# casys-kaist/CoVA

Measured on AMD Instinct MI355X. Metric: compressed-domain frames/sec (BlobNet+bboxcc) at 1080p b=256, higher is better.
Workload: dtype f16

## Files before the change

cova_amd/csrc/blobnet.h:

```cpp
#pragma once
#include <hip/hip_fp16.h>

#include <vector>

#include "internal.h"

constexpr int BN_T = 4;
constexpr int BN_LEVELS = 4;
constexpr int BN_KTAB_STACKS = 256;

struct BnLevelGeom {
    int H, W;
};

struct BnWorkspace {
    bool ready = false;
    __half *act[BN_LEVELS + 1] = {};
    __half *dact[BN_LEVELS] = {};
    __half *pbuf = nullptr;
    size_t pbuf_frames = 0;
    float *part = nullptr;
    int32_t *d_index = nullptr;
    int32_t *h_index = nullptr;
    size_t index_ints = 0;
// ... 6 lines not shown
    hipEvent_t ev_models = nullptr;
    std::vector<uint8_t> last_models;
    int32_t *d_areas = nullptr;
    int32_t *h_areas = nullptr;
    size_t areas_cap = 0;
    hipEvent_t ev_areas = nullptr;
    std::vector<int32_t> last_areas;
};

struct covahip_blobnet {
    int H = 0, W = 0, max_batch = 0;
    int n_models = 1;
    BnLevelGeom lv[BN_LEVELS + 1];
    int enc_c[BN_LEVELS + 1] = {3, 16, 32, 64, 128};
    int dec_ci[BN_LEVELS] = {128, 128, 64, 32};
    int dec_co[BN_LEVELS] = {64, 32, 16, 16};
    int dec_cy[BN_LEVELS], dec_cx[BN_LEVELS];
    BnWorkspace ws[COVAHIP_MAX_LANES];
    void *d_prepared = nullptr;
    size_t prepared_bytes = 0;
    struct Prepared *prep = nullptr;
    int fuse_tail = 1;
    int fuse_dec = 1;
    int enc1_tile16 = 1;
    int tail_rows = 1;
    int tail_part = 1;
    int fuse_enc23 = 1;
    int enc_rowtiles = 1;
    int64_t macs_per_frame = 0;
    std::vector<float> post_thr;
    std::vector<int32_t> post_area;
    bool area_on = false;
    std::vector<std::vector<uint8_t>> post_keep;
    bool post_on = false;
    void *d_post = nullptr;
    size_t post_area_off = 0, post_keep_off = 0, post_planes_off = 0, post_keep_stride = 0, post_planes_stride = 0, post_bytes = 0;
};

constexpr int BN_E1_MAXW = 62;
inline bool bn_level1_on_enc1(const covahip_ctx *ctx, const covahip_blobnet *m) {
    return m->enc1_tile16 && m->enc_c[1] == 16 && m->enc_c[2] == 32 && m->lv[1].W <= BN_E1_MAXW && m->lv[1].H >= 2 &&
           !ctx->enc_plan[1].nbands;
}

int blobnet_prepare_mfma(covahip_ctx *ctx, covahip_blobnet *m, const float *const *h_weights, int n_models);
void blobnet_release_mfma(covahip_ctx *ctx, covahip_blobnet *m);
// ... 22 lines not shown
```

cova_amd/csrc/blobnet.hip:

```cpp
#include <algorithm>
#include <cmath>
#include <cstdlib>
#include <cstring>
#include <vector>

#include "blobnet.h"
#include "covahip_dev.h"

namespace {

constexpr uint32_t W_MAGIC = 0x57485643;
constexpr size_t N_PARAMS = 320305;

}

static void free_model(covahip_ctx *ctx, covahip_blobnet *m) {
    if (!m) return;
    blobnet_release_mfma(ctx, m);
    if (m->d_post) hipFree(m->d_post);
    for (BnWorkspace &ws : m->ws) {
        for (int i = 0; i <= BN_LEVELS; i++)
            if (ws.act[i]) hipFree(ws.act[i]);
        for (int j = 0; j < BN_LEVELS; j++)
            if (ws.dact[j]) hipFree(ws.dact[j]);
// ... 452 lines not shown
        const size_t hw = (size_t)m->H * m->W;
        if (keep.empty()) std::memset(keep_or_null, 1, hw);
        else std::memcpy(keep_or_null, keep.data(), hw);
    }
    return COVAHIP_OK;
}

int covahip_blobnet_macs_per_frame(covahip_ctx *ctx, int64_t *macs) {
    if (!ctx || !macs) return COVAHIP_ERR_INVALID_ARG;
    if (!ctx->blobnet) return COVAHIP_ERR_NOT_LOADED;
    *macs = ctx->blobnet->macs_per_frame;
    return COVAHIP_OK;
}

int covahip_blobnet_set_enc_plan(covahip_ctx *ctx, int level, int nbands, int nbuf) {
    if (!ctx || level < 1 || level > 3 || nbands < 0 || nbands > 64 || (nbands && nbuf != 1 && nbuf != 2)) return COVAHIP_ERR_INVALID_ARG;
    ctx->enc_plan[level].nbands = nbands;
    ctx->enc_plan[level].nbuf = nbands ? nbuf : 0;
    return COVAHIP_OK;
}

int covahip_blobnet_set_impl(covahip_ctx *ctx, int impl) {
    if (!ctx || !ctx->blobnet) return COVAHIP_ERR_NOT_LOADED;
    if (impl != 1 && (impl < 4 || impl > 10)) return COVAHIP_ERR_INVALID_ARG;
    ctx->blobnet->fuse_dec = impl != 4;
    ctx->blobnet->enc1_tile16 = impl != 5;
    ctx->blobnet->enc_rowtiles = impl != 6;
    ctx->blobnet->fuse_enc23 = impl == 7 ? 0 : impl == 8 ? 2 : 1;
    ctx->blobnet->tail_part = impl != 9;
    ctx->blobnet->tail_rows = impl != 10;
    return COVAHIP_OK;
}

static int filter_placed(covahip_ctx *ctx, covahip_blobnet *m, const uint8_t *d_src, int n_frames, const int32_t *stack_index,
                         int batch, int area_thresh, covahip_box *d_boxes, int32_t *d_counts, int max_boxes, float *d_logits,
                         uint8_t *d_mask, bool packed = false, const uint8_t *model_ids = nullptr) {
    if (!d_mask) {
        CtxLane &l = ctx->lane();
        int rc = covahip_ensure_buffer(ctx, &l.cc_scratch, &l.cc_scratch_bytes, (size_t)batch * m->H * m->W);
        if (rc) return rc;
        d_mask = (uint8_t *)l.cc_scratch;
    }
    BnInput in;
    if (n_frames > 0) {
        int rc = prepare_frames(ctx, m, m->ws[ctx->cur_lane], d_src, n_frames, stack_index, batch, in, model_ids);
        if (rc) return rc;
        in.packed = packed;
    } else {
        in.stack = d_src;
    }
    return filter_dev(ctx, in, batch, d_logits, d_mask, true, area_thresh, d_boxes, d_counts, max_boxes, n_frames > 0 ? nullptr : model_ids);
}

// ... 235 lines not shown
```

cova_amd/csrc/blobnet_mfma.hip:

```cpp
#include <algorithm>
#include <cmath>
#include <cstdlib>
#include <cstring>
#include <mutex>
#include <type_traits>
#include <utility>
#include <vector>

#include "bboxcc_body.h"
#include "bboxcc_wave.h"
#include "blobnet.h"
#include "covahip_dev.h"

typedef _Float16 half8 __attribute__((ext_vector_type(8)));
typedef _Float16 half4 __attribute__((ext_vector_type(4)));
typedef float f32x16 __attribute__((ext_vector_type(16)));
typedef float f32x4 __attribute__((ext_vector_type(4)));
typedef _Float16 half2v __attribute__((ext_vector_type(2)));

namespace {

constexpr float BN_EPS = 1e-3f;
constexpr int WG = 256;

// ... 1112 lines not shown
            const uint4 sv = *reinterpret_cast<const uint4 *>(scr + ll * 16);
            if (owin < nwin) {
                const int owy = fdiv(owin, p.mWp), owx = owin - owy * p.Wp;
                const int gy = y0 / 2 + owy + p.oy, gx = owx + p.ox;
                const uint32_t eo = (uint32_t)((gy * p.Wo + gx) * 32 + 8 * (m & 3));
                *reinterpret_cast<uint4 *>(ob + (m >> 2) * tstride + eo) = sv;
                if (ride && m < 4) {
                    float *const pw = reinterpret_cast<float *>(pb4 + (y0 + 2 * owy) * GW + 2 * owx) + m;
                    pw[0] = pride[0]; pw[4] = pride[1]; pw[4 * GW] = pride[2]; pw[4 * GW + 4] = pride[3];
                }
            }
            __builtin_amdgcn_fence(__ATOMIC_RELEASE, "wavefront");
            __builtin_amdgcn_wave_barrier();
            PHASE_MARK(7);
        }
    }
#ifdef PHASE_TIMING
    if (tid == 64 * (PHASE_WAVE < 0 ? NWV + PHASE_WAVE : PHASE_WAVE))
        for (int i = 0; i < 9; i++) atomicAdd(&g_phase[i], ph_[i]);
#endif
    WGSPAN_END(0);
}

constexpr int E23_RP2 = 2048;
constexpr int E23_NSLOT = 6;
constexpr int E23_TSZ2 = E23_NSLOT * E23_RP2;
struct Enc23Args {
    const __half *in;
    __half *mid;
    __half *out;
    const half8 *wf2, *wf3;
    const float *epi2, *epi3;
    int B;
    int H2, W2, Hp2, Wp2;
    int H3, W3, Hp3, Wp3, oy3, ox3;
    int H4, W4, oy4, ox4;
    Swz swz2, swz3;
    int ring_off, xchg_off, scr_off;
    const uint8_t *model_ids;
    uint32_t mstride;
};
template <bool AP2, bool AP3, bool MS = false>
__global__ __launch_bounds__(512, 2) void enc23_mfma(Enc23Args p) {
    extern __shared__ __attribute__((aligned(256))) uint8_t smem[];
    WGSPAN_BEGIN();
    const int tid = threadIdx.x, lane = tid & 63;
    const int wave = __builtin_amdgcn_readfirstlane(tid >> 6);
    uint8_t *const ring = smem + p.ring_off;
    uint8_t *const xchg = smem + p.xchg_off;
    const int TC3 = p.W3 + 2;
    bool first = true;
    const int tc2 = wave & 1, nt2 = (wave >> 1) & 1, th = wave >> 2;
    const int nt3 = wave & 3, mg3 = wave >> 2;
    for (int b = blockIdx.x; b < p.B; b += gridDim.x) {
        [[maybe_unused]] const uint32_t moff = model_off<MS>(p.model_ids, p.mstride, b);
        int ll = lane;
        asm volatile("" : "+v"(ll));
        lds_barrier();
        const uint8_t *const src_b = reinterpret_cast<const uint8_t *>(p.in) + (size_t)b * BN_T * p.H2 * p.W2 * 64;
        const int st_t = tid >> 7, st_i = tid & 127, st_c = st_i >> 2, st_x = st_c - 1;
        const bool st_xin = st_x >= 0 && st_x < p.W2;
        uint32_t st_so[2];
#pragma unroll
        for (int k = 0; k < 2; k++)
            st_so[k] = (uint32_t)((min(max(st_x, 0), p.W2 - 1)) * 64 + (((st_i & 3) ^ swz_eval<4>(p.swz2, st_c, k)) << 4));
// ... 5 lines not shown
                const int rc = min(max(r0 + k, 0), p.H2 - 1);
                v[k] = *reinterpret_cast<const uint4 *>(st_src + (size_t)rc * p.W2 * 64 + st_so[k]);
            }
        };
        auto store_rows = [&](int r0, const uint4 (&v)[2]) {
#pragma unroll
            for (int k = 0; k < 2; k++) {
                const int row = r0 + k;
                const bool in = st_xin && row >= 0 && row < p.H2;
                *reinterpret_cast<uint4 *>(st_dst + ((row + 1) % E23_NSLOT) * E23_RP2) = in ? v[k] : make_uint4(0, 0, 0, 0);
            }
        };
        {
            uint4 va[2], vb[2];
            load_rows(-1, va);
            load_rows(1, vb);
            if (first) {
                for (int i = tid; i < BN_T * E3_TSZ / 16; i += 512) *reinterpret_cast<uint4 *>(smem + i * 16) = make_uint4(0, 0, 0, 0);
                first = false;
            }
            store_rows(-1, va);
            store_rows(1, vb);
        }
        {
            const int m0 = ll & 31, kh = ll >> 5;
            const int yl = (m0 >> 1) & 1, xl = 2 * (m0 >> 2) + (m0 & 1);
            uint32_t xq2[9];
#pragma unroll
            for (int tap = 0; tap < 9; tap++) {
                const int yy = yl + tap / 3, xx = xl + 16 * tc2 + tap % 3;
                xq2[tap] = (uint32_t)(p.ring_off + th * 2 * E23_TSZ2 + xx * 64) ^ (uint32_t)((kh ^ swz_eval<4>(p.swz2, xx, yy)) << 4);
            }
            half8 bf[18];
            {
                const half8 *wp = at_model(p.wf2, moff) + nt2 * 18 * 64 + ll;
                asm volatile("" : "+v"(wp));
#pragma unroll
                for (int ks = 0; ks < 18; ks++) bf[ks] = wp[ks * 64];
            }
            const int co = nt2 * 32 + (ll & 31);
            const float *const epi2 = at_model(p.epi2, moff);
            const float e0 = epi2[co], e1 = epi2[64 + co], e2 = epi2[128 + co];
            const TmixW tm = load_tmix(epi2 + 192, ll);
            int s0 = 0;
            for (int s = 0; s < p.Hp2; s++) {
                lds_barrier();
                uint4 vn[2];
                const bool pre = s + 1 < p.Hp2;
                if (pre) load_rows(2 * s + 3, vn);
                uint32_t fa[9];
                {
#pragma unroll
                    for (int ty = 0; ty < 3; ty++) {
                        int slot = s0 + ty + yl;
                        slot = slot >= E23_NSLOT ? slot - E23_NSLOT : slot;
                        const uint32_t rr = (uint32_t)(slot * E23_RP2);
#pragma unroll
                        for (int tx = 0; tx < 3; tx++) fa[ty * 3 + tx] = xq2[ty * 3 + tx] + rr;
                    }
                }
                s0 = s0 + 2 >= E23_NSLOT ? s0 + 2 - E23_NSLOT : s0 + 2;
                constexpr int AD = 8, NS = 36;
                auto frag = [&](int i) -> half8 {
                    const int tap = i >> 2, kc = (i >> 1) & 1, t = i & 1;
                    const uint8_t *a = smem + (fa[tap] ^ (uint32_t)(kc << 5));
                    return *reinterpret_cast<const half8 *>(__builtin_assume_aligned(a + t * E23_TSZ2, 16));
                };
                half8 ab[AD];
#pragma unroll
                for (int i = 0; i < AD; i++) ab[i] = frag(i);
                f32x16 acc[2];
#pragma unroll
                for (int i = 0; i < NS; i++) {
                    const int t = i & 1;
                    if (i < 2) {
#pragma unroll
                        for (int q = 0; q < 16; q++) acc[t][q] = 0.f;
                    }
                    acc[t] = __builtin_amdgcn_mfma_f32_32x32x16_f16(ab[i % AD], bf[i >> 1], acc[t], 0, 0, 0);
                    if (i + AD < NS) ab[i % AD] = frag(i + AD);
                }
                __builtin_amdgcn_sched_group_barrier(0x100, AD, 0);
#pragma unroll
                for (int i = 0; i < NS; i++) {
                    __builtin_amdgcn_sched_group_barrier(0x008, 1, 0);
                    if (i + AD < NS) __builtin_amdgcn_sched_group_barrier(0x100, 1, 0);
                }
                half2v hp[4];
#pragma unroll
                for (int g = 0; g < 4; g++)
#pragma unroll
                    for (int t = 0; t < 2; t++)
                        hp[g][t] = (_Float16)pool4<AP2>(acc[t][4 * g], acc[t][4 * g + 1], acc[t][4 * g + 2], acc[t][4 * g + 3], e0, e1, e2);
                {
                    typedef _Float16 half4x __attribute__((ext_vector_type(4)));
                    const half4x give = th ? half4x{hp[0][0], hp[0][1], hp[1][0], hp[1][1]} : half4x{hp[2][0], hp[2][1], hp[3][0], hp[3][1]};
                    *reinterpret_cast<half4x *>(xchg + (wave * 64 + ll) * 8) = give;
                }
                if (pre) store_rows(2 * s + 3, vn);
                lds_barrier();
                half4 pb[2], o[2];
                {
                    const half4 got = *reinterpret_cast<const half4 *>(xchg + ((wave ^ 4) * 64 + ll) * 8);
                    if (th == 0) {
                        pb[0] = half4{hp[0][0], hp[0][1], got[0], got[1]};
                        pb[1] = half4{hp[1][0], hp[1][1], got[2], got[3]};
                    } else {
                        pb[0] = half4{got[0], got[1], hp[2][0], hp[2][1]};
                        pb[1] = half4{got[2], got[3], hp[3][0], hp[3][1]};
                    }
                }
                tmix4h<2>(tm, pb, o);
#pragma unroll
                for (int gl = 0; gl < 2; gl++) {
                    const int owx = 8 * tc2 + 2 * (2 * th + gl) + kh;
                    if (owx < p.Wp2) {
                        const int yy = s + p.oy3 + 1, xx = owx + p.ox3 + 1;
                        uint8_t *d = smem + (yy * TC3 + xx) * 128 + ((((co >> 3) ^ swz_eval<8>(p.swz3, xx, yy))) << 4) + (co & 7) * 2;
#pragma unroll
                        for (int t = 0; t < BN_T; t++) *reinterpret_cast<_Float16 *>(d + t * E3_TSZ) = o[gl][t];
                    }
                }
            }
        }
        {
            int l3 = lane;
            asm volatile("" : "+v"(l3));
            const int m0 = l3 & 31, kh = l3 >> 5;
            const int yl = (m0 >> 1) & 1, xl = 2 * (m0 >> 2) + (m0 & 1);
            half8 bf[36];
            {
                const half8 *wp = at_model(p.wf3, moff) + nt3 * 36 * 64 + ll;
                asm volatile("" : "+v"(wp));
#pragma unroll
                for (int ks = 0; ks < 36; ks++) bf[ks] = wp[ks * 64];
            }
            lds_barrier();
            {
                __half *const mb = p.mid + (size_t)b * BN_T * p.H3 * p.W3 * 64;
                const int npc = p.Hp2 * p.Wp2 * 8;
                for (int i = tid; i < npc; i += 512) {
                    const int pix = i >> 3, j = i & 7;
                    const int wy = pix / p.Wp2, wx = pix - wy * p.Wp2;
                    const int yy = wy + p.oy3 + 1, xx = wx + p.ox3 + 1;
                    const uint4 v = *reinterpret_cast<const uint4 *>(smem + (yy * TC3 + xx) * 128 + ((j ^ swz_eval<8>(p.swz3, xx, yy)) << 4));
                    *reinterpret_cast<uint4 *>(mb + ((size_t)(yy - 1) * p.W3 + (xx - 1)) * 64 + j * 8) = v;
                }
            }
            const int co = nt3 * 32 + (ll & 31);
            const float *const epi3 = at_model(p.epi3, moff);
            const float e0 = epi3[co], e1 = epi3[128 + co], e2 = epi3[256 + co];
            const TmixW tm = load_tmix(epi3 + 384, ll);
            uint32_t kq[9];
#pragma unroll
            for (int tap = 0; tap < 9; tap++) {
                const int yy = yl + tap / 3, xx = xl + tap % 3;
                kq[tap] = (uint32_t)((yy * TC3 + xx) * 128) ^ (uint32_t)((kh ^ swz_eval<8>(p.swz3, xx, yy)) << 4);
            }
// ... 274 lines not shown
template <int C1, int C2>
__device__ __forceinline__ void dec012_stage(uint8_t *tile, const __half *ss, const DecLvl &g, int wave, int lane, int first) {
    constexpr int C = C1 + C2, CPP = C / 8;
    const int RC = (g.Wi + 2) * CPP, NI = g.Wi * CPP;
    for (int y = (wave + 8 - first) & 7; y < g.Hi; y += 8) {
        const int r = y + 1;
        const __half *rowp = ss + (size_t)y * g.Wi * C2;
        uint8_t *rowl = tile + (r * RC + CPP) * 16;
        for (int q0 = 0; q0 < NI; q0 += 64) {
            const int q = q0 + lane;
            const int px = q / CPP, chp = q % CPP;
            const int cb = (chp ^ swz_eval<CPP>(g.swz, px + 1, r)) * 8;
            if (q < NI && cb >= C1) glds16(rowp + px * C2 + (cb - C1), rowl + q0 * 16);
        }
    }
}

template <int C, int COUT>
struct Dec012W {
    half8 wf[4 * (C / 16)];
    float es[16], eb[16];
};
template <int C, int COUT>
__device__ __forceinline__ void dec012_load(Dec012W<C, COUT> &w, const half8 *wfrag, const float *epi, int wave, int lane) {
    constexpr int MT = 4 * COUT / 32, KSTEPS = 4 * (C / 16);
    const int mtile = wave % MT, kh = lane >> 5;
    asm volatile("" : "+s"(wfrag), "+s"(epi));
#pragma unroll
    for (int ks = 0; ks < KSTEPS; ks++) w.wf[ks] = wfrag[(mtile * KSTEPS + ks) * 64 + lane];
#pragma unroll
    for (int gq = 0; gq < 4; gq++) {
        const int c0 = (mtile * 32 + 8 * gq + 4 * kh) % COUT;
        const float4 sc = *reinterpret_cast<const float4 *>(epi + c0), sh = *reinterpret_cast<const float4 *>(epi + COUT + c0);
        w.es[4 * gq] = sc.x; w.es[4 * gq + 1] = sc.y; w.es[4 * gq + 2] = sc.z; w.es[4 * gq + 3] = sc.w;
        w.eb[4 * gq] = sh.x; w.eb[4 * gq + 1] = sh.y; w.eb[4 * gq + 2] = sh.z; w.eb[4 * gq + 3] = sh.w;
    }
}
template <int C1, int C2, int COUT, int CN>
__device__ __forceinline__ void dec012_block(const uint8_t *lds0, const uint8_t *tile, uint8_t *next_tile, __half *gout, uint8_t *scr_base,
                                             const Dec012W<C1 + C2, COUT> &w, const DecLvl &g, const DecLvl &gn,
                                             int wave, int lane) {
    constexpr int C = C1 + C2, MT = 4 * COUT / 32, PG = 8 / MT;
    constexpr int KC = C / 16, KSTEPS = 4 * KC, CPP = C / 8, PS = C * 2;
    constexpr int AD = C == 128 ? 4 : 8;
    const int mtile = wave % MT, pgroup = wave / MT;
    const int TC = g.Wi + 2, GW = g.Wi + 1, GH = g.Hi + 1;
    const int kh = lane >> 5;
    const half8 (&wf)[KSTEPS] = w.wf;
    const float (&es)[16] = w.es, (&eb)[16] = w.eb;
    const int npos = GH * GW;
    const int ntiles = (npos + 31) / 32;
    for (int tile_i = pgroup; tile_i < ntiles; tile_i += PG) {
        const int q = tile_i * 32 + (lane & 31);
        const int qc = min(q, npos - 1);
        const int u = fdiv(qc, g.mGW), v = qc - u * GW;
        const uint32_t toff = (uint32_t)(uintptr_t)(lds_void *)tile;
        uint32_t pk[4];
#pragma unroll
// ... 3 lines not shown
        }
        auto frag = [&](int ks) -> half8 {
            const int tp = ks / KC, kc = ks % KC;
            typedef const __attribute__((address_space(3))) half8 *lds_half8_ptr;
            return *(lds_half8_ptr)(uintptr_t)(pk[tp] ^ (uint32_t)(kc << 5));
        };
        half8 ring[AD];
#pragma unroll
        for (int ks = 0; ks < AD; ks++) ring[ks] = frag(ks);
        f32x16 acc;
#pragma unroll
        for (int r = 0; r < 16; r++) acc[r] = 0.f;
#pragma unroll
        for (int ks = 0; ks < KSTEPS; ks++) {
            acc = __builtin_amdgcn_mfma_f32_32x32x16_f16(wf[ks], ring[ks % AD], acc, 0, 0, 0);
            if (ks + AD < KSTEPS) ring[ks % AD] = frag(ks + AD);
        }
        __builtin_amdgcn_sched_group_barrier(0x100, AD, 0);
#pragma unroll
        for (int ks = 0; ks < KSTEPS; ks++) {
            __builtin_amdgcn_sched_group_barrier(0x008, 1, 0);
            if (ks + AD < KSTEPS) __builtin_amdgcn_sched_group_barrier(0x100, 1, 0);
        }
        if constexpr (CN > 0) {
            constexpr int CPPN = CN / 8, PSN = CN * 2;
            const int TCN = gn.Wi + 2;
            static_assert(COUT >= 32 && COUT % 32 == 0, "one output pixel per lane and tile");
            const int nb = mtile * 32 + 4 * kh;
            const int phase = nb / COUT, cob = nb % COUT;
            const int Y = 2 * u + (phase >> 1) - g.cy, X = 2 * v + (phase & 1) - g.cx;
            if (q < npos && Y >= 0 && Y < g.Hd && X >= 0 && X < g.Wd) {
                const int yy = Y + 1, xx = X + 1;
                uint8_t *const pix = next_tile + (yy * TCN + xx) * PSN + (cob & 7) * 2;
                const int sw = swz_eval<CPPN>(gn.swz, xx, yy);
#pragma unroll
                for (int gq = 0; gq < 4; gq++) {
                    half4 o;
#pragma unroll
                    for (int j = 0; j < 4; j++)
                        o[j] = (_Float16)fmaxf(acc[4 * gq + j] * es[4 * gq + j] + eb[4 * gq + j], 0.f);
                    *reinterpret_cast<half4 *>(pix + ((((cob >> 3) + gq) ^ sw) * 16)) = o;
                }
            }
        } else {
            uint8_t *const scr = scr_base + wave * 2048;
            const int pos = lane & 31;
#pragma unroll
            for (int gq = 0; gq < 4; gq++) {
                half4 o;
#pragma unroll
                for (int j = 0; j < 4; j++) o[j] = (_Float16)fmaxf(acc[4 * gq + j] * es[4 * gq + j] + eb[4 * gq + j], 0.f);
                *reinterpret_cast<half4 *>(scr + pos * 64 + ((gq ^ ((pos >> 2) & 3)) * 16) + kh * 8) = o;
            }
            __builtin_amdgcn_fence(__ATOMIC_RELEASE, "wavefront");
            __builtin_amdgcn_wave_barrier();
            __builtin_amdgcn_fence(__ATOMIC_ACQUIRE, "wavefront");
#pragma unroll
            for (int j = 0; j < 2; j++) {
                const int c = j * 64 + lane;
                const int rp = c >> 2;
                const int gq = (c & 3) ^ ((rp >> 2) & 3);
                const int rq = tile_i * 32 + rp;
                if (rq < npos) {
                    const int ru = fdiv(rq, g.mGW), rv = rq - ru * GW;
                    const int n0 = mtile * 32 + 8 * gq;
                    const int phase = n0 / COUT, co0 = n0 % COUT;
                    const int Y = 2 * ru + (phase >> 1) - g.cy, X = 2 * rv + (phase & 1) - g.cx;
                    if (Y >= 0 && Y < g.Hd && X >= 0 && X < g.Wd)
                        *reinterpret_cast<uint4 *>(gout + ((size_t)Y * g.Wd + X) * COUT + co0) =
                            *reinterpret_cast<const uint4 *>(scr + c * 16);
                }
            }
            __builtin_amdgcn_fence(__ATOMIC_RELEASE, "wavefront");
            __builtin_amdgcn_wave_barrier();
        }
    }
}

template <bool MS = false>
__global__ __launch_bounds__(512, 2) void dec012_mfma(Dec012Args p) {
    extern __shared__ __attribute__((aligned(256))) uint8_t smem[];
    const int tid = threadIdx.x, lane = tid & 63, wave = tid >> 6;
    uint8_t *const t0 = smem + p.lv[0].tile_off, *const t1 = smem + p.lv[1].tile_off, *const t2 = smem + p.lv[2].tile_off;
    WGSPAN_BEGIN();
#ifdef PHASE_TIMING
    unsigned long long ph_[9] = {0, 0, 0, 0, 0, 0, 0, 0, 0}, last_ = __builtin_amdgcn_s_memrealtime();
#endif
    dec012_zero_border<128>(t0, p.lv[0], tid);
    dec012_zero_border<128>(t1, p.lv[1], tid);
    dec012_zero_border<64>(t2, p.lv[2], tid);
    for (int b = blockIdx.x; b < p.B; b += gridDim.x) {
        [[maybe_unused]] const uint32_t moff = model_off<MS>(p.model_ids, p.mstride, b);
        if (b != (int)blockIdx.x) lds_barrier();
        PHASE_MARK(0);
        {
            Dec012W<128, 64> w0;
            dec012_load(w0, at_model(p.wf[0], moff), at_model(p.epi[0], moff), wave, lane);
            dec012_stage<0, 128>(t0, p.skip[0] + (size_t)b * p.Ts[0] * p.lv[0].Hi * p.lv[0].Wi * 128, p.lv[0], wave, lane, 0);
            dec012_stage<64, 64>(t1, p.skip[1] + (size_t)b * p.Ts[1] * p.lv[1].Hi * p.lv[1].Wi * 64, p.lv[1], wave, lane, p.lv[0].Hi & 7);
            dec012_stage<32, 32>(t2, p.skip[2] + (size_t)b * p.Ts[2] * p.lv[2].Hi * p.lv[2].Wi * 32, p.lv[2], wave, lane,
                                 (p.lv[0].Hi + p.lv[1].Hi) & 7);
            PHASE_MARK(1);
            wait_vmem();
            lds_barrier();
            PHASE_MARK(2);
            dec012_block<0, 128, 64, 128>(smem, t0, t1, nullptr, nullptr, w0, p.lv[0], p.lv[1], wave, lane);
        }
        PHASE_MARK(3);
        {
            Dec012W<128, 32> w1;
            dec012_load(w1, at_model(p.wf[1], moff), at_model(p.epi[1], moff), wave, lane);
            lds_barrier();
#ifdef PHASE_TIMING
            asm volatile("s_waitcnt vmcnt(0)" ::: "memory");
#endif
            PHASE_MARK(4);
            dec012_block<64, 64, 32, 64>(smem, t1, t2, nullptr, nullptr, w1, p.lv[1], p.lv[2], wave, lane);
        }
        PHASE_MARK(5);
        {
            Dec012W<64, 16> w2;
            dec012_load(w2, at_model(p.wf[2], moff), at_model(p.epi[2], moff), wave, lane);
            lds_barrier();
#ifdef PHASE_TIMING
            asm volatile("s_waitcnt vmcnt(0)" ::: "memory");
#endif
            PHASE_MARK(6);
            dec012_block<32, 32, 16, 0>(smem, t2, nullptr, p.out + (size_t)b * p.lv[2].Hd * p.lv[2].Wd * 16, smem + p.scr_off, w2,
                                        p.lv[2], p.lv[2], wave, lane);
        }
        PHASE_MARK(7);
    }
#ifdef PHASE_TIMING
    if (tid == 0)
        for (int i = 0; i < 9; i++) atomicAdd(&g_phase[48 + i], ph_[i]);
#endif
    WGSPAN_END(3);
}

struct Dec3ccArgs {
    DecArgs d;
    ccbody::CcGeom g;
    ccwave::WvGeom wg;
    int use_wv;
    covahip_box *boxes;
    int32_t *counts;
    int area_thresh, max_boxes;
    int tile_bytes;
    int mfull_off, cc_off;
    int part_off;
    DecMs ms;
};
// ... 798 lines not shown
    const Prepared *pr = f.pr;
    if (!(m->fuse_enc23 && m->enc_rowtiles && !f.ctx->enc_plan[2].nbands && !f.ctx->enc_plan[3].nbands && m->enc_c[2] == 32 &&
          m->enc_c[3] == 64 && m->enc_c[4] == 128))
        return false;
    const int H = m->lv[2].H, W = m->lv[2].W, Hp = H / 2, Wp = W / 2;
    const int H3 = m->lv[3].H, W3 = m->lv[3].W, Hp3 = H3 / 2, Wp3 = W3 / 2;
    const size_t lds = (size_t)BN_T * E3_TSZ + (size_t)BN_T * E23_TSZ2 + 4096;
    const bool pays = 4 * f.batch >= 3 * f.num_cu && 20 * Wp >= 17 * 8 * ((Wp + 7) / 8) && 20 * Wp3 >= 17 * 8 * ((Wp3 + 7) / 8);
    if (!((pays || m->fuse_enc23 == 2 || f.ms) && (W + 2) * 64 <= E23_RP2 && Wp <= 16 && Hp >= 1 && Hp3 >= 1 && Wp3 >= 1 &&
          (size_t)std::max(2 * Hp3 + 2, H3 + 1) * (W3 + 2) * 128 <= (size_t)E3_TSZ && lds <= 160 * 1024 - 256))
        return false;
    Enc23Args a;
    a.in = f.ws.act[2]; a.mid = f.ws.act[3]; a.out = f.ws.act[4];
    a.wf2 = (const half8 *)(f.prep + pr->enc[2].wfrag); a.wf3 = (const half8 *)(f.prep + pr->enc[3].wfrag);
    a.epi2 = (const float *)(f.prep + pr->enc[2].epi); a.epi3 = (const float *)(f.prep + pr->enc[3].epi);
    a.B = f.batch;
    a.H2 = H; a.W2 = W; a.Hp2 = Hp; a.Wp2 = Wp;
    a.H3 = H3; a.W3 = W3; a.Hp3 = Hp3; a.Wp3 = Wp3; a.oy3 = H & 1; a.ox3 = W & 1;
    a.H4 = m->lv[4].H; a.W4 = m->lv[4].W; a.oy4 = H3 & 1; a.ox4 = W3 & 1;
    a.swz2 = choose_swz_periodic(32, 30, Wp); a.swz3 = choose_swz_periodic(64, W3, Wp3);
    a.ring_off = BN_T * E3_TSZ; a.xchg_off = a.ring_off + BN_T * E23_TSZ2; a.scr_off = a.ring_off;
    a.model_ids = f.inp.model_ids; a.mstride = f.mstride;
    const int grid = std::min(f.batch, f.num_cu);
    rc = launched(f, with_bools([&](auto AP2, auto AP3, auto MS) {
        return launch(f, "enc23_mfma", enc23_mfma<AP2.value, AP3.value, MS.value>, grid, 512, lds, a);
    }, pr->allpos[2], pr->allpos[3], f.ms));
    return true;
}

int run_enc_level(const Fwd &f, int i) {
    const covahip_blobnet *m = f.m;
    const Prepared *pr = f.pr;
    const int H = m->lv[i].H, W = m->lv[i].W, Hp = H / 2, Wp = W / 2;
    const int cin = m->enc_c[i];
    const size_t px_bytes = (size_t)cin * 2;
    const int TC = W + 2;
    static const int enc_waves[BN_LEVELS] = {0, 8, 4, 8};
    int nbuf = 1, wgs_per_cu = (i == BN_LEVELS - 1) ? 1 : 2;
    int nbands = 0;
    const size_t scr_bytes = (size_t)enc_waves[i] * 2048;
    if (f.ctx->enc_plan[i].nbands) {
        nbands = std::min(f.ctx->enc_plan[i].nbands, Hp);
        nbuf = f.ctx->enc_plan[i].nbuf;
        const size_t need = (size_t)nbuf * BN_T * (2 * ((Hp + nbands - 1) / nbands) + 2) * TC * px_bytes + scr_bytes;
        if (need > 160 * 1024 - 256) return COVAHIP_ERR_UNSUPPORTED;
        wgs_per_cu = (i == BN_LEVELS - 1) ? 1 : (int)std::min<size_t>(2, (160 * 1024 - 256) / need);
    } else {
        const size_t lds_cap = (wgs_per_cu == 1 ? 150 * 1024 : 80 * 1024) - scr_bytes;
        nbands = plan_bands(Hp, f.batch, (long long)wgs_per_cu * f.num_cu,
// ... 49 lines not shown
          m->dec_co[1] == 32 && m->dec_co[2] == 16))
        return false;
    Dec012Args a;
    size_t off = 0;
    for (int j = 0; j < 3; j++) {
        const BnLevelGeom in = m->lv[BN_LEVELS - j], out = m->lv[BN_LEVELS - 1 - j];
        DecLvl &g = a.lv[j];
        g.Hi = in.H; g.Wi = in.W; g.Hd = out.H; g.Wd = out.W; g.cy = m->dec_cy[j]; g.cx = m->dec_cx[j];
        g.mGW = magic(in.W + 1);
        g.mRC = magic((in.W + 2) * (m->dec_ci[j] / 8));
        g.swz = choose_swz(false, m->dec_ci[j], in.W, 0, in.H + 1);
        g.tile_off = (int)off;
        off += (((size_t)(in.H + 2) * (in.W + 2) * m->dec_ci[j] * 2) + 255) & ~(size_t)255;
        a.skip[j] = f.ws.act[BN_LEVELS - j];
        a.Ts[j] = j == 0 ? 1 : BN_T;
        a.wf[j] = (const half8 *)(f.prep + pr->dec[j].wfrag);
        a.epi[j] = (const float *)(f.prep + pr->dec[j].epi);
    }
    a.scr_off = (int)off;
    const size_t lds = off + 8 * 2048;
    if (lds > 160 * 1024 - 256) return false;
    a.out = f.ws.dact[2]; a.B = f.batch; a.zero = f.prep + pr->zero;
    a.model_ids = f.inp.model_ids; a.mstride = f.mstride;
    rc = launched(f, with_bools([&](auto MS) {
        return launch(f, "dec012_mfma", dec012_mfma<MS.value>, std::min(f.batch, f.num_cu), 512, lds, a);
    }, f.ms));
    return true;
}

struct DecPlan {
    DecArgs a;
    DecMs am;
    BnLevelGeom in, out;
    bool half;
    int ci, GH, grid;
    size_t row_bytes, lds;
};
int plan_dec_block(const Fwd &f, int j, DecPlan &p) {
    const covahip_blobnet *m = f.m;
    const Prepared *pr = f.pr;
    const BnLevelGeom in = m->lv[BN_LEVELS - j], out = m->lv[BN_LEVELS - 1 - j];
    const bool last = j == BN_LEVELS - 1;
    const bool half = last && f.part_written;
    const int ci_j = half ? m->dec_ci[j] / 2 : m->dec_ci[j];
    DecArgs &a = p.a;
    a.up = j == 0 ? nullptr : f.ws.dact[j - 1];
    a.skip = f.ws.act[BN_LEVELS - j];
    a.out = last ? nullptr : f.ws.dact[j];
    a.logits = last ? f.d_logits : nullptr;
// ... 188 lines not shown
```

cova_amd/elements.py:

```python
from __future__ import annotations

import ctypes as C

import numpy as np

from . import _lib as L
from . import weights as W

FLOW_OK = "ok"
FLOW_DROPPED = "dropped"


def _ptr(a: np.ndarray) -> int:
    return a.ctypes.data


def _optr(a: np.ndarray | None) -> int | None:
    return None if a is None else a.ctypes.data


class Context:

    def __init__(self, device_id: int = 0):
        self._lib = L.lib()
# ... 170 lines not shown

    def reset_post(self, model: int = 0):
        L.check(self._lib.covahip_blobnet_set_post(self.ctx.handle, model, None), "covahip_blobnet_set_post", self.ctx.handle)

    def post(self, model: int = 0):
        thr, has = C.c_float(), C.c_int()
        keep = np.empty((self.h, self.w), dtype=np.uint8)
        L.check(self._lib.covahip_blobnet_get_post(self.ctx.handle, model, C.byref(thr), _ptr(keep), C.byref(has)),
                "covahip_blobnet_get_post", self.ctx.handle)
        return thr.value, (keep if has.value else None)

    def set_area(self, model: int = 0, area: int = 0):
        L.check(self._lib.covahip_blobnet_set_area(self.ctx.handle, model, int(area)), "covahip_blobnet_set_area", self.ctx.handle)

    def get_area(self, model: int = 0) -> int:
        v = C.c_int()
        L.check(self._lib.covahip_blobnet_get_area(self.ctx.handle, model, C.byref(v)), "covahip_blobnet_get_area", self.ctx.handle)
        return v.value

    def set_enc_plan(self, level: int, nbands: int, nbuf: int = 1):
        L.check(self._lib.covahip_blobnet_set_enc_plan(self.ctx.handle, level, nbands, nbuf), "covahip_blobnet_set_enc_plan")

    def set_impl(self, impl: str):
        L.check(self._lib.covahip_blobnet_set_impl(self.ctx.handle, {"mfma": 1, "dec_separate": 4, "enc1_legacy": 5, "enc_general_tiles": 6, "enc23_separate": 7, "enc23_force": 8, "tail_skip_tensor": 9, "tail_band_tiles": 10}[impl]), "set_impl")

    TAIL_ALONE, TAIL_ROWS, TAIL_BANDS = 1, 2, 4

    def tail_form(self) -> int:
        v = C.c_int()
        L.check(self._lib.covahip_dev_blobnet_tail_form(self.ctx.handle, C.byref(v)), "covahip_dev_blobnet_tail_form")
        return v.value

    def read_buffer(self, which: int, index: int = 0) -> np.ndarray:
        p, n, dims = C.c_void_p(), C.c_size_t(), (C.c_int32 * 5)()
        L.check(self._lib.covahip_dev_blobnet_buffer(self.ctx.handle, which, index, C.byref(p), C.byref(n), dims),
                "covahip_dev_blobnet_buffer", self.ctx.handle)
        out = np.empty(tuple(d for d in dims if d), dtype=np.float32 if which == 3 else np.float16)
        assert p.value and out.nbytes == n.value, (which, index, n.value, tuple(dims))
        self.ctx.d2h(out, p.value)
        return out

    @property
    def macs_per_frame(self) -> int:
        v = C.c_int64()
        L.check(self._lib.covahip_blobnet_macs_per_frame(self.ctx.handle, C.byref(v)), "macs_per_frame")
        return v.value

# ... 526 lines not shown
```

Baseline: 2.424 million.

## Prefetch next decoder level weights into recycled registers during last tiles

In the fused decoder kernel, the weight-fragment registers of the current level are reused. While the final tiles of one level run, the next level's weight fragments are loaded into them with inline global loads, so the weight-load latency between levels is hidden. Tile processing now also handles two tiles per wave on the last pass, and the epilogue is factored into a helper. A similar register-recycling prefetch for enc23 is added behind a non-default option (impl 12). The price is fragile hand-written waitcnt and asm register pinning, plus higher register pressure.

```diff
diff --git a/cova_amd/csrc/blobnet.h b/cova_amd/csrc/blobnet.h
--- a/cova_amd/csrc/blobnet.h
+++ b/cova_amd/csrc/blobnet.h
@@ -52,6 +52,8 @@
     struct Prepared *prep = nullptr;
     int fuse_tail = 1;
     int fuse_dec = 1;
+    int dec_kouter = 1;
+    int enc23_recycle = 0;
     int enc1_tile16 = 1;
     int tail_rows = 1;
     int tail_part = 1;
diff --git a/cova_amd/csrc/blobnet.hip b/cova_amd/csrc/blobnet.hip
--- a/cova_amd/csrc/blobnet.hip
+++ b/cova_amd/csrc/blobnet.hip
@@ -498,13 +498,15 @@
 
 int covahip_blobnet_set_impl(covahip_ctx *ctx, int impl) {
     if (!ctx || !ctx->blobnet) return COVAHIP_ERR_NOT_LOADED;
-    if (impl != 1 && (impl < 4 || impl > 10)) return COVAHIP_ERR_INVALID_ARG;
+    if (impl != 1 && (impl < 4 || impl > 12)) return COVAHIP_ERR_INVALID_ARG;
     ctx->blobnet->fuse_dec = impl != 4;
     ctx->blobnet->enc1_tile16 = impl != 5;
     ctx->blobnet->enc_rowtiles = impl != 6;
-    ctx->blobnet->fuse_enc23 = impl == 7 ? 0 : impl == 8 ? 2 : 1;
+    ctx->blobnet->fuse_enc23 = impl == 7 ? 0 : impl == 8 || impl == 12 ? 2 : 1;
     ctx->blobnet->tail_part = impl != 9;
     ctx->blobnet->tail_rows = impl != 10;
+    ctx->blobnet->dec_kouter = impl != 11;
+    ctx->blobnet->enc23_recycle = impl == 12;
     return COVAHIP_OK;
 }
 
diff --git a/cova_amd/csrc/blobnet_mfma.hip b/cova_amd/csrc/blobnet_mfma.hip
--- a/cova_amd/csrc/blobnet_mfma.hip
+++ b/cova_amd/csrc/blobnet_mfma.hip
@@ -1158,6 +1158,7 @@
     WGSPAN_END(0);
 }
 
+__device__ __forceinline__ void dec012_recycle(half8 &f, uint32_t voff, const half8 *base, int ks);
 constexpr int E23_RP2 = 2048;
 constexpr int E23_NSLOT = 6;
 constexpr int E23_TSZ2 = E23_NSLOT * E23_RP2;
@@ -1176,7 +1177,7 @@
     const uint8_t *model_ids;
     uint32_t mstride;
 };
-template <bool AP2, bool AP3, bool MS = false>
+template <bool AP2, bool AP3, bool MS = false, bool RC = false>
 __global__ __launch_bounds__(512, 2) void enc23_mfma(Enc23Args p) {
     extern __shared__ __attribute__((aligned(256))) uint8_t smem[];
     WGSPAN_BEGIN();
@@ -1228,7 +1229,9 @@
             store_rows(-1, va);
             store_rows(1, vb);
         }
+        half8 bf2[18];
         {
+            half8 (&bf)[18] = bf2;
             const int m0 = ll & 31, kh = ll >> 5;
             const int yl = (m0 >> 1) & 1, xl = 2 * (m0 >> 2) + (m0 & 1);
             uint32_t xq2[9];
@@ -1237,7 +1240,6 @@
                 const int yy = yl + tap / 3, xx = xl + 16 * tc2 + tap % 3;
                 xq2[tap] = (uint32_t)(p.ring_off + th * 2 * E23_TSZ2 + xx * 64) ^ (uint32_t)((kh ^ swz_eval<4>(p.swz2, xx, yy)) << 4);
             }
-            half8 bf[18];
             {
                 const half8 *wp = at_model(p.wf2, moff) + nt2 * 18 * 64 + ll;
                 asm volatile("" : "+v"(wp));
@@ -1249,10 +1251,14 @@
             const float e0 = epi2[co], e1 = epi2[64 + co], e2 = epi2[128 + co];
             const TmixW tm = load_tmix(epi2 + 192, ll);
             int s0 = 0;
-            for (int s = 0; s < p.Hp2; s++) {
+            const half8 *wf3b = at_model(p.wf3, moff);
+            uint32_t voff3 = (uint32_t)((nt3 * 36 * 64 + ll) * 16);
+            asm volatile("" : "+s"(wf3b));
+            auto step = [&](int s, auto LAST) __attribute__((always_inline)) {
+                constexpr bool last = decltype(LAST)::value;
                 lds_barrier();
                 uint4 vn[2];
-                const bool pre = s + 1 < p.Hp2;
+                const bool pre = !last && s + 1 < p.Hp2;
                 if (pre) load_rows(2 * s + 3, vn);
                 uint32_t fa[9];
                 {
@@ -1285,12 +1291,18 @@
                     }
                     acc[t] = __builtin_amdgcn_mfma_f32_32x32x16_f16(ab[i % AD], bf[i >> 1], acc[t], 0, 0, 0);
                     if (i + AD < NS) ab[i % AD] = frag(i + AD);
-                }
-                __builtin_amdgcn_sched_group_barrier(0x100, AD, 0);
-#pragma unroll
-                for (int i = 0; i < NS; i++) {
-                    __builtin_amdgcn_sched_group_barrier(0x008, 1, 0);
-                    if (i + AD < NS) __builtin_amdgcn_sched_group_barrier(0x100, 1, 0);
+                    if (last && (i & 1)) {
+                        dec012_recycle(bf[i >> 1], voff3, wf3b, i >> 1);
+                        if (((i >> 1) & 3) == 3) voff3 += 4096;
+                    }
+                }
+                if constexpr (!last) {
+                    __builtin_amdgcn_sched_group_barrier(0x100, AD, 0);
+#pragma unroll
+                    for (int i = 0; i < NS; i++) {
+                        __builtin_amdgcn_sched_group_barrier(0x008, 1, 0);
+                        if (i + AD < NS) __builtin_amdgcn_sched_group_barrier(0x100, 1, 0);
+                    }
                 }
                 half2v hp[4];
 #pragma unroll
@@ -1327,6 +1339,12 @@
                         for (int t = 0; t < BN_T; t++) *reinterpret_cast<_Float16 *>(d + t * E3_TSZ) = o[gl][t];
                     }
                 }
+            };
+            if constexpr (RC) {
+                for (int s = 0; s + 1 < p.Hp2; s++) step(s, std::false_type{});
+                step(p.Hp2 - 1, std::true_type{});
+            } else {
+                for (int s = 0; s < p.Hp2; s++) step(s, std::false_type{});
             }
         }
         {
@@ -1339,7 +1357,14 @@
                 const half8 *wp = at_model(p.wf3, moff) + nt3 * 36 * 64 + ll;
                 asm volatile("" : "+v"(wp));
 #pragma unroll
-                for (int ks = 0; ks < 36; ks++) bf[ks] = wp[ks * 64];
+                for (int ks = RC ? 18 : 0; ks < 36; ks++) bf[ks] = wp[ks * 64];
+            }
+            if constexpr (RC) {
+                __builtin_amdgcn_s_waitcnt(0x4F72);
+                asm volatile("" : "+v"(bf2[0]), "+v"(bf2[1]), "+v"(bf2[2]), "+v"(bf2[3]), "+v"(bf2[4]), "+v"(bf2[5]), "+v"(bf2[6]), "+v"(bf2[7]), "+v"(bf2[8]));
+                asm volatile("" : "+v"(bf2[9]), "+v"(bf2[10]), "+v"(bf2[11]), "+v"(bf2[12]), "+v"(bf2[13]), "+v"(bf2[14]), "+v"(bf2[15]), "+v"(bf2[16]), "+v"(bf2[17]));
+#pragma unroll
+                for (int ks = 0; ks < 18; ks++) bf[ks] = bf2[ks];
             }
             lds_barrier();
             {
@@ -1660,18 +1685,85 @@
     float es[16], eb[16];
 };
 template <int C, int COUT>
-__device__ __forceinline__ void dec012_load(Dec012W<C, COUT> &w, const half8 *wfrag, const float *epi, int wave, int lane) {
-    constexpr int MT = 4 * COUT / 32, KSTEPS = 4 * (C / 16);
+__device__ __forceinline__ void dec012_load_epi(Dec012W<C, COUT> &w, const float *epi, int wave, int lane) {
+    constexpr int MT = 4 * COUT / 32;
     const int mtile = wave % MT, kh = lane >> 5;
-    asm volatile("" : "+s"(wfrag), "+s"(epi));
-#pragma unroll
-    for (int ks = 0; ks < KSTEPS; ks++) w.wf[ks] = wfrag[(mtile * KSTEPS + ks) * 64 + lane];
+    asm volatile("" : "+s"(epi));
 #pragma unroll
     for (int gq = 0; gq < 4; gq++) {
         const int c0 = (mtile * 32 + 8 * gq + 4 * kh) % COUT;
         const float4 sc = *reinterpret_cast<const float4 *>(epi + c0), sh = *reinterpret_cast<const float4 *>(epi + COUT + c0);
         w.es[4 * gq] = sc.x; w.es[4 * gq + 1] = sc.y; w.es[4 * gq + 2] = sc.z; w.es[4 * gq + 3] = sc.w;
         w.eb[4 * gq] = sh.x; w.eb[4 * gq + 1] = sh.y; w.eb[4 * gq + 2] = sh.z; w.eb[4 * gq + 3] = sh.w;
+    }
+}
+template <int C, int COUT>
+__device__ __forceinline__ void dec012_load(Dec012W<C, COUT> &w, const half8 *wfrag, const float *epi, int wave, int lane) {
+    constexpr int MT = 4 * COUT / 32, KSTEPS = 4 * (C / 16);
+    const int mtile = wave % MT;
+    asm volatile("" : "+s"(wfrag));
+#pragma unroll
+    for (int ks = 0; ks < KSTEPS; ks++) w.wf[ks] = wfrag[(mtile * KSTEPS + ks) * 64 + lane];
+    dec012_load_epi(w, epi, wave, lane);
+}
+template <int C1, int C2, int COUT, int CN>
+__device__ __forceinline__ void dec012_epilogue(const f32x16 &acc, int tile_i, int q, int u, int v, uint8_t *next_tile, __half *gout,
+                                                uint8_t *scr_base, const float (&es)[16], const float (&eb)[16], const DecLvl &g,
+                                                const DecLvl &gn, int wave, int lane) {
+    constexpr int MT = 4 * COUT / 32;
+    const int mtile = wave % MT, kh = lane >> 5;
+    const int GW = g.Wi + 1, npos = (g.Hi + 1) * GW;
+    if constexpr (CN > 0) {
+        constexpr int CPPN = CN / 8, PSN = CN * 2;
+        const int TCN = gn.Wi + 2;
+        static_assert(COUT >= 32 && COUT % 32 == 0, "one output pixel per lane and tile");
+        const int nb = mtile * 32 + 4 * kh;
+        const int phase = nb / COUT, cob = nb % COUT;
+        const int Y = 2 * u + (phase >> 1) - g.cy, X = 2 * v + (phase & 1) - g.cx;
+        if (q < npos && Y >= 0 && Y < g.Hd && X >= 0 && X < g.Wd) {
+            const int yy = Y + 1, xx = X + 1;
+            uint8_t *const pix = next_tile + (yy * TCN + xx) * PSN + (cob & 7) * 2;
+            const int sw = swz_eval<CPPN>(gn.swz, xx, yy);
+#pragma unroll
+            for (int gq = 0; gq < 4; gq++) {
+                half4 o;
+#pragma unroll
+                for (int j = 0; j < 4; j++)
+                    o[j] = (_Float16)fmaxf(acc[4 * gq + j] * es[4 * gq + j] + eb[4 * gq + j], 0.f);
+                *reinterpret_cast<half4 *>(pix + ((((cob >> 3) + gq) ^ sw) * 16)) = o;
+            }
+        }
+    } else {
+        uint8_t *const scr = scr_base + wave * 2048;
+        const int pos = lane & 31;
+#pragma unroll
+        for (int gq = 0; gq < 4; gq++) {
+            half4 o;
+#pragma unroll
+            for (int j = 0; j < 4; j++) o[j] = (_Float16)fmaxf(acc[4 * gq + j] * es[4 * gq + j] + eb[4 * gq + j], 0.f);
+            *reinterpret_cast<half4 *>(scr + pos * 64 + ((gq ^ ((pos >> 2) & 3)) * 16) + kh * 8) = o;
+        }
+        __builtin_amdgcn_fence(__ATOMIC_RELEASE, "wavefront");
+        __builtin_amdgcn_wave_barrier();
+        __builtin_amdgcn_fence(__ATOMIC_ACQUIRE, "wavefront");
+#pragma unroll
+        for (int j = 0; j < 2; j++) {
+            const int c = j * 64 + lane;
+            const int rp = c >> 2;
+            const int gq = (c & 3) ^ ((rp >> 2) & 3);
+            const int rq = tile_i * 32 + rp;
+            if (rq < npos) {
+                const int ru = fdiv(rq, g.mGW), rv = rq - ru * GW;
+                const int n0 = mtile * 32 + 8 * gq;
+                const int phase = n0 / COUT, co0 = n0 % COUT;
+                const int Y = 2 * ru + (phase >> 1) - g.cy, X = 2 * rv + (phase & 1) - g.cx;
+                if (Y >= 0 && Y < g.Hd && X >= 0 && X < g.Wd)
+                    *reinterpret_cast<uint4 *>(gout + ((size_t)Y * g.Wd + X) * COUT + co0) =
+                        *reinterpret_cast<const uint4 *>(scr + c * 16);
+            }
+        }
+        __builtin_amdgcn_fence(__ATOMIC_RELEASE, "wavefront");
+        __builtin_amdgcn_wave_barrier();
     }
 }
 template <int C1, int C2, int COUT, int CN>
@@ -1721,62 +1813,105 @@
             __builtin_amdgcn_sched_group_barrier(0x008, 1, 0);
             if (ks + AD < KSTEPS) __builtin_amdgcn_sched_group_barrier(0x100, 1, 0);
         }
-        if constexpr (CN > 0) {
-            constexpr int CPPN = CN / 8, PSN = CN * 2;
-            const int TCN = gn.Wi + 2;
-            static_assert(COUT >= 32 && COUT % 32 == 0, "one output pixel per lane and tile");
-            const int nb = mtile * 32 + 4 * kh;
-            const int phase = nb / COUT, cob = nb % COUT;
-            const int Y = 2 * u + (phase >> 1) - g.cy, X = 2 * v + (phase & 1) - g.cx;
-            if (q < npos && Y >= 0 && Y < g.Hd && X >= 0 && X < g.Wd) {
-                const int yy = Y + 1, xx = X + 1;
-                uint8_t *const pix = next_tile + (yy * TCN + xx) * PSN + (cob & 7) * 2;
-                const int sw = swz_eval<CPPN>(gn.swz, xx, yy);
-#pragma unroll
-                for (int gq = 0; gq < 4; gq++) {
-                    half4 o;
-#pragma unroll
-                    for (int j = 0; j < 4; j++)
-                        o[j] = (_Float16)fmaxf(acc[4 * gq + j] * es[4 * gq + j] + eb[4 * gq + j], 0.f);
-                    *reinterpret_cast<half4 *>(pix + ((((cob >> 3) + gq) ^ sw) * 16)) = o;
-                }
-            }
-        } else {
-            uint8_t *const scr = scr_base + wave * 2048;
-            const int pos = lane & 31;
-#pragma unroll
-            for (int gq = 0; gq < 4; gq++) {
-                half4 o;
-#pragma unroll
-                for (int j = 0; j < 4; j++) o[j] = (_Float16)fmaxf(acc[4 * gq + j] * es[4 * gq + j] + eb[4 * gq + j], 0.f);
-                *reinterpret_cast<half4 *>(scr + pos * 64 + ((gq ^ ((pos >> 2) & 3)) * 16) + kh * 8) = o;
-            }
-            __builtin_amdgcn_fence(__ATOMIC_RELEASE, "wavefront");
-            __builtin_amdgcn_wave_barrier();
-            __builtin_amdgcn_fence(__ATOMIC_ACQUIRE, "wavefront");
-#pragma unroll
-            for (int j = 0; j < 2; j++) {
-                const int c = j * 64 + lane;
-                const int rp = c >> 2;
-                const int gq = (c & 3) ^ ((rp >> 2) & 3);
-                const int rq = tile_i * 32 + rp;
-                if (rq < npos) {
-                    const int ru = fdiv(rq, g.mGW), rv = rq - ru * GW;
-                    const int n0 = mtile * 32 + 8 * gq;
-                    const int phase = n0 / COUT, co0 = n0 % COUT;
-                    const int Y = 2 * ru + (phase >> 1) - g.cy, X = 2 * rv + (phase & 1) - g.cx;
-                    if (Y >= 0 && Y < g.Hd && X >= 0 && X < g.Wd)
-                        *reinterpret_cast<uint4 *>(gout + ((size_t)Y * g.Wd + X) * COUT + co0) =
-                            *reinterpret_cast<const uint4 *>(scr + c * 16);
-                }
-            }
-            __builtin_amdgcn_fence(__ATOMIC_RELEASE, "wavefront");
-            __builtin_amdgcn_wave_barrier();
-        }
-    }
-}
-
-template <bool MS = false>
+        dec012_epilogue<C1, C2, COUT, CN>(acc, tile_i, q, u, v, next_tile, gout, scr_base, es, eb, g, gn, wave, lane);
+    }
+}
+
+__device__ __forceinline__ void dec012_recycle(half8 &f, uint32_t voff, const half8 *base, int ks) {
+    __builtin_amdgcn_sched_barrier(0);
+    switch (ks & 3) {
+    case 0: asm volatile("global_load_dwordx4 %0, %1, %2" : "+v"(f) : "v"(voff), "s"(base)); break;
+    case 1: asm volatile("global_load_dwordx4 %0, %1, %2 offset:1024" : "+v"(f) : "v"(voff), "s"(base)); break;
+    case 2: asm volatile("global_load_dwordx4 %0, %1, %2 offset:2048" : "+v"(f) : "v"(voff), "s"(base)); break;
+    default: asm volatile("global_load_dwordx4 %0, %1, %2 offset:3072" : "+v"(f) : "v"(voff), "s"(base)); break;
+    }
+}
+template <int N, int KEEP>
+__device__ __forceinline__ void dec012_recycled(half8 (&wf)[32]) {
+    static_assert(N % 8 == 0 && KEEP < 16, "");
+    __builtin_amdgcn_s_waitcnt(0x0F70 | KEEP);
+#pragma unroll
+    for (int i = 0; i < N; i += 8)
+        asm volatile("" : "+v"(wf[i]), "+v"(wf[i + 1]), "+v"(wf[i + 2]), "+v"(wf[i + 3]), "+v"(wf[i + 4]), "+v"(wf[i + 5]), "+v"(wf[i + 6]),
+                          "+v"(wf[i + 7]));
+}
+template <int C1, int C2, int COUT, int CN, int NT, int NKN, bool EPIX, int CX, int COUTX>
+__device__ __forceinline__ void dec012_tiles(const uint8_t *tile, uint8_t *next_tile, half8 (&wf)[32], const Dec012W<C1 + C2, COUT> &w,
+                                             Dec012W<CX, COUTX> &wx, const half8 *wfx, const float *epix, uint32_t voff, const DecLvl &g,
+                                             const DecLvl &gn, int tile0, int wave, int lane) {
+    constexpr int C = C1 + C2, MT = 4 * COUT / 32, PG = 8 / MT;
+    constexpr int KC = C / 16, KSTEPS = 4 * KC, CPP = C / 8, PS = C * 2;
+    constexpr int AD = NT == 1 ? 4 : 2;
+    static_assert(CN > 0 && KSTEPS <= 32 && NKN <= KSTEPS && NKN % 8 == 0, "");
+    const int TC = g.Wi + 2, GW = g.Wi + 1, npos = (g.Hi + 1) * GW;
+    const int kh = lane >> 5;
+    const uint32_t toff = (uint32_t)(uintptr_t)(lds_void *)tile;
+    uint32_t pk[NT][4];
+#pragma unroll
+    for (int t = 0; t < NT; t++) {
+        const int qc = min((tile0 + t * PG) * 32 + (lane & 31), npos - 1);
+        const int u = fdiv(qc, g.mGW), v = qc - u * GW;
+#pragma unroll
+        for (int tp = 0; tp < 4; tp++) {
+            const int yy = u + 1 - (tp >> 1), xx = v + 1 - (tp & 1);
+            pk[t][tp] = (toff + (uint32_t)((yy * TC + xx) * PS)) | (uint32_t)((kh ^ swz_eval<CPP>(g.swz, xx, yy)) << 4);
+        }
+    }
+    auto frag = [&](int t, int ks) -> half8 {
+        const int tp = ks / KC, kc = ks % KC;
+        typedef const __attribute__((address_space(3))) half8 *lds_half8_ptr;
+        return *(lds_half8_ptr)(uintptr_t)(pk[t][tp] ^ (uint32_t)(kc << 5));
+    };
+    half8 ring[NT][AD];
+    f32x16 acc[NT];
+#pragma unroll
+    for (int t = 0; t < NT; t++) {
+#pragma unroll
+        for (int ks = 0; ks < AD; ks++) ring[t][ks] = frag(t, ks);
+#pragma unroll
+        for (int r = 0; r < 16; r++) acc[t][r] = 0.f;
+    }
+#pragma unroll
+    for (int ks = 0; ks < KSTEPS; ks++) {
+#pragma unroll
+        for (int t = 0; t < NT; t++) {
+            acc[t] = __builtin_amdgcn_mfma_f32_32x32x16_f16(wf[ks], ring[t][ks % AD], acc[t], 0, 0, 0);
+            if (ks + AD < KSTEPS) ring[t][ks % AD] = frag(t, ks + AD);
+        }
+        if (ks < NKN) {
+            dec012_recycle(wf[ks], voff, wfx, ks);
+            if ((ks & 3) == 3) voff += 4096;
+        }
+    }
+    if constexpr (NKN > 0 && EPIX) {
+        __builtin_amdgcn_sched_barrier(0);
+        dec012_load_epi(wx, epix, wave, lane);
+    }
+#pragma unroll
+    for (int t = 0; t < NT; t++) {
+        const int tile_i = tile0 + t * PG;
+        const int q = tile_i * 32 + (lane & 31), qc = min(q, npos - 1);
+        const int u = fdiv(qc, g.mGW), v = qc - u * GW;
+        dec012_epilogue<C1, C2, COUT, CN>(acc[t], tile_i, q, u, v, next_tile, nullptr, nullptr, w.es, w.eb, g, gn, wave, lane);
+    }
+    if constexpr (NKN > 0) dec012_recycled<NKN, EPIX ? 8 : 0>(wf);
+}
+template <int C1, int C2, int COUT, int CN, bool EPIX, int CX, int COUTX>
+__device__ __forceinline__ void dec012_block_kouter(const uint8_t *tile, uint8_t *next_tile, half8 (&wf)[32], const Dec012W<C1 + C2, COUT> &w,
+                                                    Dec012W<CX, COUTX> &wx, const half8 *wfx, const float *epix, const DecLvl &g,
+                                                    const DecLvl &gn, int wave, int lane) {
+    constexpr int MT = 4 * COUT / 32, PG = 8 / MT, MTX = 4 * COUTX / 32, NKN = 4 * (CX / 16);
+    const int wv = __builtin_amdgcn_readfirstlane(wave);
+    const int ntiles = ((g.Hi + 1) * (g.Wi + 1) + 31) / 32;
+    int tile0 = wv / MT;
+    asm volatile("" : "+s"(wfx));
+    const uint32_t voff = (uint32_t)(((wave % MTX) * NKN * 64 + lane) * 16);
+    for (; tile0 + 2 * PG < ntiles; tile0 += PG)
+        dec012_tiles<C1, C2, COUT, CN, 1, 0, EPIX, CX, COUTX>(tile, next_tile, wf, w, wx, wfx, epix, voff, g, gn, tile0, wave, lane);
+    dec012_tiles<C1, C2, COUT, CN, 2, NKN, EPIX, CX, COUTX>(tile, next_tile, wf, w, wx, wfx, epix, voff, g, gn, tile0, wave, lane);
+}
+
+template <bool MS = false, bool KO = true>
 __global__ __launch_bounds__(512, 2) void dec012_mfma(Dec012Args p) {
     extern __shared__ __attribute__((aligned(256))) uint8_t smem[];
     const int tid = threadIdx.x, lane = tid & 63, wave = tid >> 6;
@@ -1792,8 +1927,13 @@
         [[maybe_unused]] const uint32_t moff = model_off<MS>(p.model_ids, p.mstride, b);
         if (b != (int)blockIdx.x) lds_barrier();
         PHASE_MARK(0);
-        {
+        if constexpr (KO) {
             Dec012W<128, 64> w0;
+            Dec012W<128, 32> w1;
+            Dec012W<64, 16> w2;
+            int tid_ = tid;
+            asm volatile("" : "+v"(tid_));
+            int lane = tid_ & 63, wave = tid_ >> 6;
             dec012_load(w0, at_model(p.wf[0], moff), at_model(p.epi[0], moff), wave, lane);
             dec012_stage<0, 128>(t0, p.skip[0] + (size_t)b * p.Ts[0] * p.lv[0].Hi * p.lv[0].Wi * 128, p.lv[0], wave, lane, 0);
             dec012_stage<64, 64>(t1, p.skip[1] + (size_t)b * p.Ts[1] * p.lv[1].Hi * p.lv[1].Wi * 64, p.lv[1], wave, lane, p.lv[0].Hi & 7);
@@ -1803,23 +1943,24 @@
             wait_vmem();
             lds_barrier();
             PHASE_MARK(2);
-            dec012_block<0, 128, 64, 128>(smem, t0, t1, nullptr, nullptr, w0, p.lv[0], p.lv[1], wave, lane);
-        }
-        PHASE_MARK(3);
-        {
-            Dec012W<128, 32> w1;
-            dec012_load(w1, at_model(p.wf[1], moff), at_model(p.epi[1], moff), wave, lane);
+            dec012_block_kouter<0, 128, 64, 128, true, 128, 32>(t0, t1, w0.wf, w0, w1, at_model(p.wf[1], moff), at_model(p.epi[1], moff), p.lv[0],
+                                                          p.lv[1], wave, lane);
+            PHASE_MARK(3);
             lds_barrier();
 #ifdef PHASE_TIMING
             asm volatile("s_waitcnt vmcnt(0)" ::: "memory");
 #endif
             PHASE_MARK(4);
-            dec012_block<64, 64, 32, 64>(smem, t1, t2, nullptr, nullptr, w1, p.lv[1], p.lv[2], wave, lane);
-        }
-        PHASE_MARK(5);
-        {
-            Dec012W<64, 16> w2;
-            dec012_load(w2, at_model(p.wf[2], moff), at_model(p.epi[2], moff), wave, lane);
+            asm volatile("" : "+v"(tid_));
+            lane = tid_ & 63, wave = tid_ >> 6;
+            dec012_block_kouter<64, 64, 32, 64, false, 64, 16>(t1, t2, w0.wf, w1, w2, at_model(p.wf[2], moff), at_model(p.epi[2], moff), p.lv[1],
+                                                        p.lv[2], wave, lane);
+            PHASE_MARK(5);
+            asm volatile("" : "+v"(tid_));
+            lane = tid_ & 63, wave = tid_ >> 6;
+            dec012_load_epi(w2, at_model(p.epi[2], moff), wave, lane);
+#pragma unroll
+            for (int ks = 0; ks < 16; ks++) w2.wf[ks] = w0.wf[ks];
             lds_barrier();
 #ifdef PHASE_TIMING
             asm volatile("s_waitcnt vmcnt(0)" ::: "memory");
@@ -1827,6 +1968,43 @@
             PHASE_MARK(6);
             dec012_block<32, 32, 16, 0>(smem, t2, nullptr, p.out + (size_t)b * p.lv[2].Hd * p.lv[2].Wd * 16, smem + p.scr_off, w2,
                                         p.lv[2], p.lv[2], wave, lane);
+        } else {
+            {
+                Dec012W<128, 64> w0;
+                dec012_load(w0, at_model(p.wf[0], moff), at_model(p.epi[0], moff), wave, lane);
+                dec012_stage<0, 128>(t0, p.skip[0] + (size_t)b * p.Ts[0] * p.lv[0].Hi * p.lv[0].Wi * 128, p.lv[0], wave, lane, 0);
+                dec012_stage<64, 64>(t1, p.skip[1] + (size_t)b * p.Ts[1] * p.lv[1].Hi * p.lv[1].Wi * 64, p.lv[1], wave, lane, p.lv[0].Hi & 7);
+                dec012_stage<32, 32>(t2, p.skip[2] + (size_t)b * p.Ts[2] * p.lv[2].Hi * p.lv[2].Wi * 32, p.lv[2], wave, lane,
+                                     (p.lv[0].Hi + p.lv[1].Hi) & 7);
+                PHASE_MARK(1);
+                wait_vmem();
+                lds_barrier();
+                PHASE_MARK(2);
+                dec012_block<0, 128, 64, 128>(smem, t0, t1, nullptr, nullptr, w0, p.lv[0], p.lv[1], wave, lane);
+            }
+            PHASE_MARK(3);
+            {
+                Dec012W<128, 32> w1;
+                dec012_load(w1, at_model(p.wf[1], moff), at_model(p.epi[1], moff), wave, lane);
+                lds_barrier();
+    #ifdef PHASE_TIMING
+                asm volatile("s_waitcnt vmcnt(0)" ::: "memory");
+    #endif
+                PHASE_MARK(4);
+                dec012_block<64, 64, 32, 64>(smem, t1, t2, nullptr, nullptr, w1, p.lv[1], p.lv[2], wave, lane);
+            }
+            PHASE_MARK(5);
+            {
+                Dec012W<64, 16> w2;
+                dec012_load(w2, at_model(p.wf[2], moff), at_model(p.epi[2], moff), wave, lane);
+                lds_barrier();
+    #ifdef PHASE_TIMING
+                asm volatile("s_waitcnt vmcnt(0)" ::: "memory");
+    #endif
+                PHASE_MARK(6);
+                dec012_block<32, 32, 16, 0>(smem, t2, nullptr, p.out + (size_t)b * p.lv[2].Hd * p.lv[2].Wd * 16, smem + p.scr_off, w2,
+                                            p.lv[2], p.lv[2], wave, lane);
+            }
         }
         PHASE_MARK(7);
     }
@@ -2671,9 +2849,9 @@
     a.ring_off = BN_T * E3_TSZ; a.xchg_off = a.ring_off + BN_T * E23_TSZ2; a.scr_off = a.ring_off;
     a.model_ids = f.inp.model_ids; a.mstride = f.mstride;
     const int grid = std::min(f.batch, f.num_cu);
-    rc = launched(f, with_bools([&](auto AP2, auto AP3, auto MS) {
-        return launch(f, "enc23_mfma", enc23_mfma<AP2.value, AP3.value, MS.value>, grid, 512, lds, a);
-    }, pr->allpos[2], pr->allpos[3], f.ms));
+    rc = launched(f, with_bools([&](auto AP2, auto AP3, auto MS, auto RC) {
+        return launch(f, "enc23_mfma", enc23_mfma<AP2.value, AP3.value, MS.value, RC.value>, grid, 512, lds, a);
+    }, pr->allpos[2], pr->allpos[3], f.ms, m->enc23_recycle != 0));
     return true;
 }
 
@@ -2769,9 +2947,9 @@
     if (lds > 160 * 1024 - 256) return false;
     a.out = f.ws.dact[2]; a.B = f.batch; a.zero = f.prep + pr->zero;
     a.model_ids = f.inp.model_ids; a.mstride = f.mstride;
-    rc = launched(f, with_bools([&](auto MS) {
-        return launch(f, "dec012_mfma", dec012_mfma<MS.value>, std::min(f.batch, f.num_cu), 512, lds, a);
-    }, f.ms));
+    rc = launched(f, with_bools([&](auto MS, auto KO) {
+        return launch(f, "dec012_mfma", dec012_mfma<MS.value, KO.value>, std::min(f.batch, f.num_cu), 512, lds, a);
+    }, f.ms, m->dec_kouter != 0));
     return true;
 }
 
diff --git a/cova_amd/elements.py b/cova_amd/elements.py
--- a/cova_amd/elements.py
+++ b/cova_amd/elements.py
@@ -216,7 +216,7 @@
         L.check(self._lib.covahip_blobnet_set_enc_plan(self.ctx.handle, level, nbands, nbuf), "covahip_blobnet_set_enc_plan")
 
     def set_impl(self, impl: str):
-        L.check(self._lib.covahip_blobnet_set_impl(self.ctx.handle, {"mfma": 1, "dec_separate": 4, "enc1_legacy": 5, "enc_general_tiles": 6, "enc23_separate": 7, "enc23_force": 8, "tail_skip_tensor": 9, "tail_band_tiles": 10}[impl]), "set_impl")
+        L.check(self._lib.covahip_blobnet_set_impl(self.ctx.handle, {"mfma": 1, "dec_separate": 4, "enc1_legacy": 5, "enc_general_tiles": 6, "enc23_separate": 7, "enc23_force": 8, "tail_skip_tensor": 9, "tail_band_tiles": 10, "dec012_tile_by_tile": 11, "enc23_recycle": 12}[impl]), "set_impl")
 
     TAIL_ALONE, TAIL_ROWS, TAIL_BANDS = 1, 2, 4
 
```

Result: no change. 2.444 million, median of 6 (+0.8%).
